# BorealisAI/noise_flow

Measured on AMD Instinct MI355X. Metric: patches/sec (32x32x4) fwd-NLL and inverse-sample; mean NLL vs CPU ref, higher is better.
Workload: dtype f32

## Files before the change

### noise_flow_amd/csrc/nf_device.h

```cpp
#pragma once
#include <stdint.h>

#define NF_MAX_OPS 64

enum : int32_t {
    NF_OP_MIX          = 1,
    NF_OP_COUPLING_FWD = 2,
    NF_OP_COUPLING_REV = 3,
    NF_OP_SDN_DIV      = 4,
    NF_OP_SDN_MUL      = 5,
    NF_OP_SCALE        = 6,
    NF_OP_SCALE_COND   = 7,
    NF_OP_STORE        = 8,
};

struct NfOp {
    int32_t type;
    int32_t off;
};

struct NfProgram {
    int32_t n_ops;
    int32_t width;
    NfOp ops[NF_MAX_OPS];
// ... 8 lines not shown
__host__ __device__ constexpr int nf_cpl_off_S(int w)  { return 64 + 36 * w + 18 * w + 2 * w + w * w; }
__host__ __device__ constexpr int nf_cpl_size(int w)   { return 64 + 36 * w + 18 * w + 2 * w + w * w + 4; }

#define NF2_MIX_SIZE 16
#define NF2_CPL_E 0
#define NF2_CPL_B1 64
#define NF2_CPL_B2 68
#define NF2_CPL_S 72
#define NF2_CPL_W1T 76
#define NF2_CPL_W2T 172
#define NF2_CPL_W3T 188
#define NF2_CPL_SIZE 332
#define NF2_MAX_FLOATS 6144

#define NF3_CPL_E 0
#define NF3_CPL_B1 64
#define NF3_CPL_B2 68
#define NF3_CPL_S 72
#define NF3_CPL_W1H 76
#define NF3_CPL_W2H 172
#define NF3_CPL_W3H 180
#define NF3_W3H_STRIDE 20
#define NF3_CPL_SIZE 260

#define NF11_CPL_E 0
#define NF11_CPL_B1 64
#define NF11_CPL_B2 68
#define NF11_CPL_S 72
#define NF11_CPL_W2H 76
#define NF11_CPL_A1 84
#define NF11_CPL_A3 340
#define NF11_CPL_SIZE 852
#define NF11_CPL_A2 852
#define NF11_CPL_SIZE_L2 1364
#define NF11_MAX_FLOATS 12288
__host__ __device__ constexpr int nf11_l1_row(int gk) { return 2 * (gk & 1) + (gk >> 1); }
__host__ __device__ constexpr int nf11_l3_row(int gk, int m3) { return 2 * (gk & 1) + m3; }
#ifndef NF11_PITCH64
#define NF11_PITCH64 80
#endif
__host__ __device__ constexpr int nf11_pitch(int side) { return side == 64 ? NF11_PITCH64 : 48; }

#define NF12_CPL_E 0
#define NF12_CPL_B1 64
#define NF12_CPL_B2 68
#define NF12_CPL_S 72
#define NF12_CPL_W2T 76
#define NF12_CPL_AOFF 92
#define NF12_CPL_SIZE 96
#define NF12_A_A1 0
#define NF12_A_A3 1536
#define NF12_A_SIZE 3072
#define NF12_PITCH 34
__host__ __device__ constexpr int nf12_col(int n) { return ((n + 12) & 15) < 8 ? 2 * ((n + 12) & 15) : 2 * (((n + 12) & 15) - 8) + 1; }
#define NF12_MAX_FLOATS 2048

#define NF4_CPL_E 0
#define NF4_CPL_S 64
#define NF4_CPL_IMG 68
#define NF4_IMG_A1 0
#define NF4_IMG_B1 768
#define NF4_IMG_A2 800
#define NF4_IMG_B2 1824
#define NF4_IMG_A3 1856
#define NF4_IMG_A3C 2880
#define NF4_IMG_SIZE 3008
#define NF4_CPL_SIZE (NF4_CPL_IMG + NF4_IMG_SIZE)
__host__ __device__ constexpr int nf4_chan(int v, int g) { return 8 * (v >> 2) + 4 * g + (v & 3); }

#define NF6_IMG_A1 0
#define NF6_IMG_B1 320
#define NF6_IMG_A2 336
#define NF6_IMG_B2 592
#define NF6_IMG_A3A 608
#define NF6_IMG_A3B 864
#define NF6_IMG_A3C 1120
#define NF6_IMG_SIZE 1184
#define NF6_CPL_SIZE (NF4_CPL_IMG + NF6_IMG_SIZE)

#define NF5_IMG_A1H 0
#define NF5_IMG_B1 512
#define NF5_IMG_A2H 544
#define NF5_IMG_B2 1056
#define NF5_IMG_A3H 1088
#define NF5_IMG_A3CH 1600
#define NF5_IMG_SIZE 1664
#define NF5_CPL_SIZE (NF4_CPL_IMG + NF5_IMG_SIZE)

#define NF7_CPL_E 0
#define NF7_CPL_S 64
#define NF7_CPL_IMG 68
__host__ __device__ constexpr int nf7_pad_width(int w) { return w <= 64 ? 64 : w <= 128 ? 128 : w <= 256 ? 256 : 512; }
__host__ __device__ constexpr int nf7_img_A1(int) { return 0; }
__host__ __device__ constexpr int nf7_img_B1(int wp) { return (wp / 32) * 768; }
__host__ __device__ constexpr int nf7_img_B2(int wp) { return (wp / 32) * 800; }
__host__ __device__ constexpr int nf7_img_A2(int wp) { return (wp / 32) * 832; }
__host__ __device__ constexpr int nf7_img_A3(int wp) { return (wp / 32) * 832 + wp * wp; }
__host__ __device__ constexpr int nf7_img_A3C(int wp) { return (wp / 32) * 832 + wp * wp + (wp / 32) * 1024; }
__host__ __device__ constexpr int nf7_img_size(int wp) { return (wp / 32) * 832 + wp * wp + (wp / 32) * (1024 + 128); }
#define NF7_P_STRIDE 44
__host__ __device__ constexpr int nf7_cpl_size(int wp) { return NF7_CPL_IMG + nf7_img_size(wp); }
#define NF7_BAND_FLOATS 32768
#define NF7_MAX_PIXELS 4096

enum : uint32_t {
    NF_K_PRIOR     = 1u,
    NF_K_PHILOX_IN = 2u,
    NF_K_FP16_CNN  = 4u,
// ... 76 lines not shown
```

### noise_flow_amd/csrc/nf_kernels.hip

```cpp
#include <hip/hip_runtime.h>
#include <math.h>
#include <stdlib.h>
#include <atomic>
#include "../../include/noiseflow_hip.h"
#include "nf_device.h"
#include "nf_dev_util.h"

#ifndef NF_PRIO
#define NF_PRIO 2
#endif
#ifndef NF_BR_SWIZZLE
#define NF_BR_SWIZZLE 1
#endif
#ifndef NF_WAVE_PRIO
#define NF_WAVE_PRIO 1
#endif
#ifndef NF_FAIR
#define NF_FAIR 1
#endif
#if NF_FAIR
#define NF_PRIO_UP()   do { } while (0)
#define NF_PRIO_DOWN() do { } while (0)
#else
#define NF_PRIO_UP()   do { if (NF_PRIO) __builtin_amdgcn_s_setprio(NF_PRIO); } while (0)
// ... 16 lines not shown
#define NF_STAMP(i) do { } while (0)
#endif

namespace {

template <int WIDTH>
__device__ __forceinline__ void stats_accumulate(const float (&h)[WIDTH], bool active, float (&s1)[WIDTH], float (&s2)[WIDTH])
{
#pragma unroll
    for (int j = 0; j < WIDTH; ++j) {
        const float v = active ? h[j] : 0.0f;
        s1[j] += v;
        s2[j] = fmaf(v, v, s2[j]);
    }
}
template <int WIDTH>
__device__ __forceinline__ void stats_direct(const float (&h)[WIDTH], bool active, double *stats, int t)
{
#pragma unroll
    for (int j = 0; j < WIDTH; ++j) {
        const float v = active ? h[j] : 0.0f;
        const float s = wave_sum(v), q = wave_sum(v * v);
        if ((t & 63) == 0) {
            atomicAdd(&stats[j], (double)s);
            atomicAdd(&stats[WIDTH + j], (double)q);
        }
    }
}
template <int WIDTH>
__device__ __forceinline__ void stats_flush(const float (&s1)[WIDTH], const float (&s2)[WIDTH], double *stats, int t)
{
#pragma unroll
    for (int j = 0; j < WIDTH; ++j) {
        const float s = wave_sum(s1[j]), q = wave_sum(s2[j]);
        if ((t & 63) == 0) {
            atomicAdd(&stats[j], (double)s);
            atomicAdd(&stats[WIDTH + j], (double)q);
        }
    }
}

__device__ __forceinline__ void nf_split3(float x0, float x1, uint32_t &h, uint32_t &m, uint32_t &l)
{
    const nf_v2bf ph = {(__bf16)x0, (__bf16)x1};
    x0 -= (float)ph[0];
    x1 -= (float)ph[1];
    const nf_v2bf pm = {(__bf16)x0, (__bf16)x1};
    x0 -= (float)pm[0];
    x1 -= (float)pm[1];
    const nf_v2bf pl = {(__bf16)x0, (__bf16)x1};
    h = __builtin_bit_cast(uint32_t, ph);
    m = __builtin_bit_cast(uint32_t, pm);
    l = __builtin_bit_cast(uint32_t, pl);
}
__device__ __forceinline__ v4f nf_mfma_bf16(const uint4 a, const uint4 b, const v4f c)
{
    return __builtin_amdgcn_mfma_f32_16x16x32_bf16(__builtin_bit_cast(nf_v8bf, a), __builtin_bit_cast(nf_v8bf, b), c, 0, 0, 0);
}

template <int WIDTH, int THREADS, int PX, bool PHILOX, bool MFMA, bool FULL, int PREC, bool BS, bool TF>
__device__ __forceinline__ void nf_flow_body(const NfProgram &prog, const NfLaunch &a)
{
    static_assert(!BS || (MFMA && PREC == 0), "the batch-statistics variant is the fp32 matrix-core kernel");
    static_assert(!TF || (FULL && MFMA && PX == 4 && PREC != 1 && !BS), "tiled full-geometry launches: the fp32 matrix-core kernel and the fp16-CNN kernel on v_mfma_f32_16x16x32_f16");
    static_assert(WIDTH % 4 == 0, "WIDTH must be a multiple of 4");
    static_assert(!MFMA || WIDTH == 4, "the matrix-core path is the width-4 specialisation");
    static_assert(PREC == 0 || (MFMA && FULL && PX == 4), "the fp16-CNN mode exists for full 2x2-blocked patches only");
    static_assert(PREC != 3 || (THREADS == 256 && !TF && !BS), "the split-bf16 mode exists for full 32x32 patches only");
    constexpr bool H16 = PREC == 1;
    constexpr bool HB = PREC == 2;
    constexpr bool SB = PREC == 3;
    constexpr bool HALF = PREC == 1 || PREC == 2;
    extern __shared__ __attribute__((aligned(16))) float smem[];

    constexpr int SIDE = THREADS * PX == 1024 ? 32 : THREADS * PX == 4096 ? 64 : 0;
    static_assert(!FULL || SIDE != 0, "FULL needs a 32x32 or 64x64 workgroup footprint");
    const int H = FULL ? SIDE : a.H, W = FULL ? SIDE : a.W, HW = H * W;
    const int Wp = SB ? NF12_PITCH : HB ? nf11_pitch(SIDE) : (H16 && SIDE == 32) ? 48 : W + 2;
    const int tile_px = ((H + 2) * Wp + 1) & ~1;
    [[maybe_unused]] const int ident_off = (a.n_params + 3) & ~3;
    constexpr bool WFIRST = HB || SB;
    constexpr int TILE_WORDS = SB ? 6 : HALF ? 3 : 2 + WIDTH;
    constexpr int RED_WORDS = (6 * (THREADS / 64) + 3) & ~3;
    float *const tiles = WFIRST ? smem + ident_off + 16 : smem;
    float2 *const t0 = reinterpret_cast<float2 *>(tiles);
    float *const th = tiles + 2 * tile_px;
    uint32_t *const t0h = reinterpret_cast<uint32_t *>(tiles);
    uint2 *const thh = reinterpret_cast<uint2 *>(tiles + tile_px);
    [[maybe_unused]] uint2 *const sr0 = reinterpret_cast<uint2 *>(tiles);
    [[maybe_unused]] uint2 *const sr1 = reinterpret_cast<uint2 *>(tiles + 2 * tile_px);
    [[maybe_unused]] uint2 *const sr2 = reinterpret_cast<uint2 *>(tiles + 4 * tile_px);
    float *const red = tiles + TILE_WORDS * tile_px;
    float *const wl = WFIRST ? smem : red + RED_WORDS;
    [[maybe_unused]] float *const bs_part = WFIRST ? red + RED_WORDS : wl + ident_off + 16;

    const int t = threadIdx.x;
    const int j4 = t & 3;
    [[maybe_unused]] bool stamp_on = true;
    [[maybe_unused]] int64_t stamp_it = 0;
    NF_STAMP(0);

    constexpr bool BLK = MFMA && FULL && PX == 4;
    const int PW = (W >> 1) + 1;
    int lidx[PX];
    int gidx[PX];
    int bmask[PX];
    bool act[PX];
    bool own[PX];
    [[maybe_unused]] int prow[PX], pcol[PX];
    int wbase = 0;
    [[maybe_unused]] int wbase3 = 0;
    if constexpr (HB || SB) {
        const int wv = t >> 6, g = (t >> 4) & 3;
        const int n = SB ? nf12_col(t & 15) : (t & 15);
        const int q = SIDE == 64 ? (wv & 1) : 0, band = SIDE == 64 ? (wv >> 1) : wv;
        const int c = 32 * q + 2 * n + (g & 1);
        wbase = (band * 8 + nf11_l1_row(g)) * Wp + 32 * q + 2 * n;
        wbase3 = (band * 8 + nf11_l3_row(g, 0)) * Wp + 32 * q + 2 * n + 2 * (g >> 1);
#pragma unroll
        for (int k = 0; k < PX; ++k) {
            const int r = band * 8 + 2 * k + (g >> 1);
            act[k] = true;
            own[k] = true;
            prow[k] = r;
            pcol[k] = c;
            gidx[k] = r * W + c;
            lidx[k] = (r + 1) * Wp + (c + 1);
            bmask[k] = (r == 0 ? 1 : 0) | (r == H - 1 ? 2 : 0) | (c == 0 ? 4 : 0) | (c == W - 1 ? 8 : 0);
        }
    } else if constexpr (BLK) {
        const int bw = W >> 1;
        int br = t / bw, bc = t - br * bw;
#if NF_BR_SWIZZLE
        if (!H16 && bw == 16) {
            br = (t >> 6) + 4 * ((t >> 4) & 3);
            bc = t & 15;
        }
#endif
        wbase = H16 ? (2 * br) * Wp + 2 * bc : (2 * br * 2) * PW + bc;
#pragma unroll
        for (int k = 0; k < PX; ++k) {
            const int dy = k >> 1, dx = k & 1;
            const int r = 2 * br + dy, c = 2 * bc + dx;
            act[k] = true;
            own[k] = true;
            prow[k] = r;
            pcol[k] = c;
            gidx[k] = r * W + c;
            lidx[k] = H16 ? (r + 1) * Wp + (c + 1) : wbase + ((dy + 1) * 2 + ((dx + 1) & 1)) * PW + ((dx + 1) >> 1);
            bmask[k] = (r == 0 ? 1 : 0) | (r == H - 1 ? 2 : 0) | (c == 0 ? 4 : 0) | (c == W - 1 ? 8 : 0);
        }
    } else {
#pragma unroll
        for (int k = 0; k < PX; ++k) {
            const int p = t + THREADS * k;
            act[k] = FULL || p < HW;
            own[k] = act[k];
            const int pp = act[k] ? p : 0;
            const int r = pp / W, c = pp - r * W;
            prow[k] = r;
            pcol[k] = c;
            gidx[k] = pp;
            lidx[k] = (r + 1) * Wp + (c + 1);
            bmask[k] = (r == 0 ? 1 : 0) | (r == H - 1 ? 2 : 0) | (c == 0 ? 4 : 0) | (c == W - 1 ? 8 : 0);
        }
    }

#ifndef NF_WSTAGE
#define NF_WSTAGE 1
#endif
    constexpr int WU = MFMA && NF_WSTAGE ? (THREADS >= 1024 ? 3 : 6) : 1;
    [[maybe_unused]] float4 wreg[WU];
    if constexpr (MFMA && NF_WSTAGE) {
        const int np4 = a.n_params >> 2;
        const float4 *const p4 = reinterpret_cast<const float4 *>(a.params);
#pragma unroll
        for (int u = 0; u < WU; ++u) {
            const int i = t + u * THREADS;
            wreg[u] = p4[i < np4 ? i : 0];
        }
    }

    float warm = 0.0f;
    float4 zin[PX];
#pragma unroll
    for (int k = 0; k < PX; ++k) zin[k] = make_float4(0.f, 0.f, 0.f, 0.f);
#ifndef NF_YPF
#define NF_YPF 1
#endif
    constexpr bool YPF = NF_YPF && MFMA && FULL && !PHILOX && THREADS == 1024 && !TF && !BS && (PREC != 0 || NF_YPF > 1);
    [[maybe_unused]] float4 yin[YPF ? PX : 1];
    [[maybe_unused]] const bool sdn_first = YPF && a.y && prog.n_ops > 0 && prog.ops[0].type == NF_OP_SDN_DIV;
    if constexpr (YPF) {
#pragma unroll
        for (int k = 0; k < PX; ++k) yin[k] = make_float4(1.f, 1.f, 1.f, 1.f);
    }
#ifndef NF_STAGGER
#define NF_STAGGER 2
#endif
#ifndef NF_STAGGER_SLEEP
#define NF_STAGGER_SLEEP 16
#endif
    const bool early = !NF_STAGGER || PHILOX || blockIdx.x < (NF_STAGGER >= 2 ? (gridDim.x >> 2) : (gridDim.x >> 1));
    bool tiled = TF;
    if constexpr (!FULL) tiled = (a.flags & NF_K_TILED) != 0;
    if ((int64_t)blockIdx.x < a.B && early && !tiled) {
        const size_t off0 = (size_t)blockIdx.x * (size_t)HW;
        if constexpr (!PHILOX) {
#pragma unroll
            for (int k = 0; k < PX; ++k)
                if (act[k]) zin[k] = reinterpret_cast<const float4 *>(a.in)[off0 + gidx[k]];
        }
        if constexpr (YPF) {
            if (sdn_first) {
#pragma unroll
                for (int k = 0; k < PX; ++k) yin[k] = reinterpret_cast<const float4 *>(a.y)[off0 + gidx[k]];
            }
        } else {
#ifndef NF_NO_WARM
#pragma unroll
        for (int k = 0; k < PX; k += NF_WARM_STEP)
            if (a.y && act[k]) warm += reinterpret_cast<const float *>(a.y)[4 * (off0 + gidx[k])];
#endif
        }
    }

    {
#ifndef NF_ZERO_BORDER
#define NF_ZERO_BORDER 0
#endif
#ifndef NF_HB_ZB
#define NF_HB_ZB 1
#endif
        if constexpr (NF_ZERO_BORDER && BLK && !HALF) {
            const int nb = 2 * (W + 2) + 2 * H;
            for (int i = t; i < nb; i += THREADS) {
                int rp, cp;
                if (i < W + 2) {
                    rp = 0;
                    cp = i;
                } else if (i < 2 * (W + 2)) {
                    rp = H + 1;
                    cp = i - (W + 2);
                } else {
                    const int j = i - 2 * (W + 2);
                    rp = 1 + (j >> 1);
                    cp = (j & 1) ? W + 1 : 0;
                }
                const int e = (rp * 2 + (cp & 1)) * PW + (cp >> 1);
                t0[e] = make_float2(0.f, 0.f);
                *reinterpret_cast<float4 *>(th + (size_t)e * 4) = make_float4(0.f, 0.f, 0.f, 0.f);
            }
        } else if constexpr (SB) {
            const int nb = 2 * (W + 2) + 2 * H;
            for (int i = t; i < nb; i += THREADS) {
                int rp, cp;
                if (i < W + 2) {
                    rp = 0;
                    cp = i;
                } else if (i < 2 * (W + 2)) {
                    rp = H + 1;
                    cp = i - (W + 2);
                } else {
                    const int j = i - 2 * (W + 2);
                    rp = 1 + (j >> 1);
                    cp = (j & 1) ? W + 1 : 0;
                }
                sr0[rp * Wp + cp] = make_uint2(0u, 0u);
                sr1[rp * Wp + cp] = make_uint2(0u, 0u);
                sr2[rp * Wp + cp] = make_uint2(0u, 0u);
            }
        } else if constexpr (NF_HB_ZB && HB) {
            const int nb = 2 * (W + 2) + 2 * H;
            for (int i = t; i < nb; i += THREADS) {
                int rp, cp;
                if (i < W + 2) {
                    rp = 0;
                    cp = i;
                } else if (i < 2 * (W + 2)) {
                    rp = H + 1;
                    cp = i - (W + 2);
                } else {
                    const int j = i - 2 * (W + 2);
                    rp = 1 + (j >> 1);
                    cp = (j & 1) ? W + 1 : 0;
                }
                t0h[rp * Wp + cp] = 0u;
                thh[rp * Wp + cp] = make_uint2(0u, 0u);
            }
        } else {
        const int nz4 = (tile_px * TILE_WORDS) >> 2;
        float4 *const s4 = reinterpret_cast<float4 *>(tiles);
        for (int i = t; i < nz4; i += THREADS) s4[i] = make_float4(0.f, 0.f, 0.f, 0.f);
        for (int i = (nz4 << 2) + t; i < tile_px * TILE_WORDS; i += THREADS) tiles[i] = 0.0f;
        }
        if (MFMA) {
            const int np4 = a.n_params >> 2;
            const float4 *const p4 = reinterpret_cast<const float4 *>(a.params);
            float4 *const w4 = reinterpret_cast<float4 *>(wl);
            if constexpr (NF_WSTAGE) {
#pragma unroll
                for (int u = 0; u < WU; ++u) {
                    const int i = t + u * THREADS;
                    if (i < np4) w4[i] = wreg[u];
                }
                for (int i = t + WU * THREADS; i < np4; i += THREADS) w4[i] = p4[i];
            } else {
                for (int i = t; i < np4; i += THREADS) w4[i] = p4[i];
            }
            for (int i = (np4 << 2) + t; i < a.n_params; i += THREADS) wl[i] = a.params[i];
            if (t < 16) wl[ident_off + t] = (t >> 2) == (t & 3) ? 1.0f : 0.0f;
        }
    }
    __syncthreads();
    asm volatile("" ::"v"(warm));
    if (NF_STAGGER && !early && (int64_t)blockIdx.x < a.B && !tiled) {
#if NF_STAGGER >= 2
        {
            const int q = (int)((blockIdx.x * 4u) / gridDim.x);
            if (q == 2) __builtin_amdgcn_s_sleep(NF_STAGGER_SLEEP);
            if (q == 3) { __builtin_amdgcn_s_sleep(NF_STAGGER_SLEEP); __builtin_amdgcn_s_sleep(NF_STAGGER_SLEEP); }
        }
#endif
        const size_t off0 = (size_t)blockIdx.x * (size_t)HW;
// ... 111 lines not shown
                const int nt = a.tile_ny * a.tile_nx;
                const int64_t img = b / nt;
                const int ti = (int)(b - img * nt);
                const int ty = ti / a.tile_nx, tx = ti - ty * a.tile_nx;
                const int oy = nf_tile_origin(ty, a.img_H, H, a.tile_halo), ox = nf_tile_origin(tx, a.img_W, W, a.tile_halo);
                const int cy0 = nf_tile_core0(ty, a.img_H, H, a.tile_halo), cy1 = nf_tile_core1(ty, a.tile_ny, a.img_H, H, a.tile_halo);
                const int cx0 = nf_tile_core0(tx, a.img_W, W, a.tile_halo), cx1 = nf_tile_core1(tx, a.tile_nx, a.img_W, W, a.tile_halo);
                patch_off = (size_t)img * (size_t)a.img_H * (size_t)a.img_W * 4u;
                patch_id = img;
#pragma unroll
                for (int k = 0; k < PX; ++k) {
                    const int r = oy + prow[k], c = ox + pcol[k];
                    gidx[k] = act[k] ? r * a.img_W + c : 0;
                    bmask[k] = (r == 0 ? 1 : 0) | (r == a.img_H - 1 ? 2 : 0) | (c == 0 ? 4 : 0) | (c == a.img_W - 1 ? 8 : 0);
                    own[k] = act[k] && r >= cy0 && r < cy1 && c >= cx0 && c < cx1;
                }
                if constexpr (!PHILOX) {
                    const float4 *in4 = reinterpret_cast<const float4 *>(a.in + patch_off);
#pragma unroll
                    for (int k = 0; k < PX; ++k) {
                        float4 v = make_float4(0.f, 0.f, 0.f, 0.f);
                        if (act[k]) v = in4[gidx[k]];
                        zin[k] = v;
                    }
                }
            }
        }

        float z[PX][4];
        if (PHILOX) {
#pragma unroll
            for (int k = 0; k < PX; ++k) {
                philox_normal4(a.seed, a.patch_base + patch_id, (uint32_t)gidx[k], NF_STREAM_SAMP, z[k]);
#pragma unroll
                for (int c = 0; c < 4; ++c) z[k][c] *= a.in_scale;
            }
        } else {
#pragma unroll
            for (int k = 0; k < PX; ++k) {
                z[k][0] = zin[k].x * a.in_scale;
                z[k][1] = zin[k].y * a.in_scale;
                z[k][2] = zin[k].z * a.in_scale;
                z[k][3] = zin[k].w * a.in_scale;
            }
        }

        float ld = 0.0f;
        if constexpr (!MFMA || BS) {
            if (a.flags & NF_K_CARRY_IN) ld = a.ld_carry[(size_t)b * THREADS + t];
        }
        float ld2 = 0.0f;
        [[maybe_unused]] int n_cpl = 0;
        [[maybe_unused]] int cpl_seen = 0;

        [[maybe_unused]] auto mix_load = [&](int moff) { return *reinterpret_cast<const float4 *>(wl + moff + 4 * j4); };
        [[maybe_unused]] auto mix_apply = [&](const float4 m) {
#pragma unroll
            for (int k = 0; k < PX; ++k) {
                v4f acc = {0.f, 0.f, 0.f, 0.f};
                acc = __builtin_amdgcn_mfma_f32_4x4x1f32(m.x, z[k][0], acc, 0, 0, 0);
                acc = __builtin_amdgcn_mfma_f32_4x4x1f32(m.y, z[k][1], acc, 0, 0, 0);
                acc = __builtin_amdgcn_mfma_f32_4x4x1f32(m.z, z[k][2], acc, 0, 0, 0);
                acc = __builtin_amdgcn_mfma_f32_4x4x1f32(m.w, z[k][3], acc, 0, 0, 0);
#pragma unroll
                for (int j = 0; j < 4; ++j) z[k][j] = acc[j];
            }
        };
        [[maybe_unused]] auto mix_mfma = [&](int mop) { mix_apply(mix_load(prog.ops[mop].off)); };

        auto sdn_apply = [&](int stype, int slot, const float4 (&yv)[PX]) {
            const float ck1 = a.cond_a[slot & 3], cb2 = a.cond_b[slot & 3];
#pragma unroll
            for (int k = 0; k < PX; ++k) {
                const float yy[4] = {yv[k].x, yv[k].y, yv[k].z, yv[k].w};
#ifndef NF_SDN_1LOG
#define NF_SDN_1LOG 1
#endif
                float rp = 1.0f;
#pragma unroll
                for (int c = 0; c < 4; ++c) {
                    const float v = fmaf(yy[c], ck1, cb2);
                    if (stype == NF_OP_SDN_DIV) {
                        const float r = __builtin_amdgcn_rsqf(v);
                        z[k][c] = z[k][c] * r;
                        if (NF_SDN_1LOG) rp = c == 0 ? r : rp * r;
                        else if (own[k]) ld = fmaf(-0.34657359027997264f, __builtin_amdgcn_logf(v), ld);
                    } else {
                        z[k][c] = z[k][c] * __builtin_amdgcn_sqrtf(v);
                    }
                }
                if (NF_SDN_1LOG && stype == NF_OP_SDN_DIV && own[k]) ld = fmaf(0.6931471805599453f, __builtin_amdgcn_logf(rp), ld);
            }
        };
        int op_begin = 0;
        if constexpr (YPF) {
            if (sdn_first) {
                float4 yv[PX];
#pragma unroll
                for (int k = 0; k < PX; ++k) yv[k] = yin[k];
                sdn_apply(NF_OP_SDN_DIV, prog.ops[0].off, yv);
                op_begin = 1;
            }
        }

        for (int op = op_begin; op < n_ops; ++op) {
            int type = prog.ops[op].type;
// ... 4 lines not shown
                    if (n_cpl == 0) { asm volatile("" ::"v"(z[0][0])); NF_STAMP(2); }
#endif
                    if (op == run_first) {
                        pr_n = run_n; pr_moff = run_moff; pr_coff = run_coff; pr_stride = run_stride;
                        type = run_type;
                    } else {
                        const int nt = op + 1 < n_ops ? prog.ops[op + 1].type : 0;
                        if (nt != NF_OP_COUPLING_FWD && nt != NF_OP_COUPLING_REV) {
                            mix_mfma(op);
                            continue;
                        }
                        pr_moff = prog.ops[op].off;
                        pr_coff = prog.ops[op + 1].off;
                        type = nt;
                    }
                    ++op;
                } else if (type == NF_OP_COUPLING_FWD || type == NF_OP_COUPLING_REV) {
                    pr_moff = ident_off;
                    pr_coff = prog.ops[op].off;
                }
            }
            [[maybe_unused]] int coff = prog.ops[op].off;
            cfloat_p P = (cfloat_p)(a.params + coff);

            if (type == NF_OP_MIX) {
                if constexpr (!MFMA) {
                    float m[16];
#pragma unroll
                    for (int i = 0; i < 16; ++i) m[i] = P[i];
#pragma unroll
                    for (int k = 0; k < PX; ++k) {
                        float o[4];
#pragma unroll
                        for (int j = 0; j < 4; ++j) {
                            float s = z[k][0] * m[j];
                            s = fmaf(z[k][1], m[4 + j], s);
                            s = fmaf(z[k][2], m[8 + j], s);
                            s = fmaf(z[k][3], m[12 + j], s);
                            o[j] = s;
                        }
#pragma unroll
                        for (int j = 0; j < 4; ++j) z[k][j] = o[j];
                    }
                }
            } else if (type == NF_OP_COUPLING_FWD || type == NF_OP_COUPLING_REV) {
                bool patch_done = false;
                synced = true;
                if constexpr (MFMA) op -= 2;
#ifndef NF_MIX_AHEAD
#define NF_MIX_AHEAD 0
#endif
                [[maybe_unused]] float4 mix_m = make_float4(0.f, 0.f, 0.f, 0.f);
                if constexpr (MFMA) mix_m = mix_load(pr_moff);
#pragma nounroll
                for (int pr_i = 0; pr_i < pr_n; ++pr_i) {
                if constexpr (MFMA) {
                    if (!NF_MIX_AHEAD) mix_m = mix_load(pr_moff);
                    mix_apply(mix_m);
                    coff = pr_coff;
                    pr_moff += pr_i + 1 < pr_n ? pr_stride : 0;
                    pr_coff += pr_stride;
                    op += 2;
                }
#if NF_FAIR
                if constexpr (MFMA && !(NF_WAVE_PRIO && THREADS == 1024)) {
                    const int lvl = (cpl_seen >= fair_t1 ? 1 : 0) + (cpl_seen >= fair_t2 ? 1 : 0) + (cpl_seen >= fair_t3 ? 1 : 0);
                    ++cpl_seen;
                    if (lvl == 0) __builtin_amdgcn_s_setprio(3);
                    else if (lvl == 1) __builtin_amdgcn_s_setprio(2);
                    else if (lvl == 2) __builtin_amdgcn_s_setprio(1);
                    else __builtin_amdgcn_s_setprio(0);
                }
#endif
#ifndef NF_HB_EARLY
#define NF_HB_EARLY 1
#endif
                [[maybe_unused]] v8h hb_a1, hb_a3a, hb_a3b, hb_a2a, hb_a2b;
                [[maybe_unused]] v4h hb_w2h;
#ifndef NF_HB_L2BIG
#define NF_HB_L2BIG 1
#endif
                constexpr bool L2B = NF_HB_L2BIG && HB && THREADS == 1024;
                [[maybe_unused]] float4 hb_b1, hb_b2, hb_e[PX];
                [[maybe_unused]] uint4 sb_a1[6], sb_a3[6];
                [[maybe_unused]] const uint4 *sb_ag = nullptr;
                if constexpr (SB) {
                    const int aoff = __builtin_amdgcn_readfirstlane(__builtin_bit_cast(int, wl[coff + NF12_CPL_AOFF]));
                    sb_ag = reinterpret_cast<const uint4 *>(a.params + aoff) + (t & 63);
#pragma unroll
                    for (int q = 0; q < 6; ++q) sb_a1[q] = sb_ag[NF12_A_A1 / 4 + 64 * q];
                    hb_b1 = *reinterpret_cast<const float4 *>(wl + coff + NF12_CPL_B1);
                    hb_b2 = *reinterpret_cast<const float4 *>(wl + coff + NF12_CPL_B2);
                }
                if constexpr (HB) {
                    const float *wb = wl + coff;
                    const uint32_t *wbw = reinterpret_cast<const uint32_t *>(wb);
                    if (NF_HB_EARLY) {
                        hb_b1 = *reinterpret_cast<const float4 *>(wb + NF11_CPL_B1);
                        hb_b2 = *reinterpret_cast<const float4 *>(wb + NF11_CPL_B2);
                        hb_a1 = __builtin_bit_cast(v8h, *reinterpret_cast<const uint4 *>(wbw + NF11_CPL_A1 + (t & 63) * 4));
                        if constexpr (L2B) {
                            hb_a2a = __builtin_bit_cast(v8h, *reinterpret_cast<const uint4 *>(wbw + NF11_CPL_A2 + (t & 63) * 4));
                            hb_a2b = __builtin_bit_cast(v8h, *reinterpret_cast<const uint4 *>(wbw + NF11_CPL_A2 + 256 + (t & 63) * 4));
                        } else {
                            hb_w2h = *reinterpret_cast<const v4h *>(wbw + NF11_CPL_W2H + j4 * 2);
                        }
                    }
                }
                if constexpr (SB) __syncthreads();
#pragma unroll
                for (int k = 0; k < PX; ++k) {
                    if constexpr (SB) {
                        uint32_t zh, zm, zl;
                        nf_split3(z[k][0], z[k][1], zh, zm, zl);
                        sr0[lidx[k]] = make_uint2(zh, zm);
                        sr1[lidx[k]] = make_uint2(zl, zh);
                    } else if constexpr (HALF) {
                        const v2h zh = {(_Float16)z[k][0], (_Float16)z[k][1]};
                        t0h[lidx[k]] = __builtin_bit_cast(uint32_t, zh);
                    } else {
                        if (act[k]) t0[lidx[k]] = make_float2(z[k][0], z[k][1]);
                    }
                }
                __syncthreads();

                if constexpr (SB) {
                    const float4 b1 = hb_b1, b2 = hb_b2;
                    const float4 w2 = *reinterpret_cast<const float4 *>(wl + coff + NF12_CPL_W2T + 4 * j4);
                    v4f h1[PX];
#pragma unroll
                    for (int k = 0; k < PX; ++k) {
                        const uint4 q00 = *reinterpret_cast<const uint4 *>(sr0 + wbase + 2 * k * Wp);
                        const uint4 q01 = *reinterpret_cast<const uint4 *>(sr0 + wbase + 2 * k * Wp + 2);
                        const uint4 q10 = *reinterpret_cast<const uint4 *>(sr1 + wbase + 2 * k * Wp);
                        const uint4 q11 = *reinterpret_cast<const uint4 *>(sr1 + wbase + 2 * k * Wp + 2);
                        v4f acc = v4f{b1.x, b1.y, b1.z, b1.w};
                        acc = nf_mfma_bf16(sb_a1[4], q10, acc);
                        acc = nf_mfma_bf16(sb_a1[5], q11, acc);
                        acc = nf_mfma_bf16(sb_a1[2], q00, acc);
                        acc = nf_mfma_bf16(sb_a1[3], q01, acc);
                        acc = nf_mfma_bf16(sb_a1[0], q00, acc);
                        acc = nf_mfma_bf16(sb_a1[1], q01, acc);
                        h1[k] = acc;
                    }
#pragma unroll
                    for (int q = 0; q < 6; ++q) sb_a3[q] = sb_ag[NF12_A_A3 / 4 + 64 * q];
                    uint2 hs[PX][3];
#pragma unroll
                    for (int k = 0; k < PX; ++k) {
                        v4f h2 = {b2.x, b2.y, b2.z, b2.w};
                        h2 = __builtin_amdgcn_mfma_f32_4x4x1f32(w2.x, nf_relu(h1[k][0]), h2, 0, 0, 0);
                        h2 = __builtin_amdgcn_mfma_f32_4x4x1f32(w2.y, nf_relu(h1[k][1]), h2, 0, 0, 0);
                        h2 = __builtin_amdgcn_mfma_f32_4x4x1f32(w2.z, nf_relu(h1[k][2]), h2, 0, 0, 0);
                        h2 = __builtin_amdgcn_mfma_f32_4x4x1f32(w2.w, nf_relu(h1[k][3]), h2, 0, 0, 0);
                        uint32_t p01[3], p23[3];
                        nf_split3(nf_relu(h2[0]), nf_relu(h2[1]), p01[0], p01[1], p01[2]);
                        nf_split3(nf_relu(h2[2]), nf_relu(h2[3]), p23[0], p23[1], p23[2]);
#pragma unroll
                        for (int q = 0; q < 3; ++q) hs[k][q] = make_uint2(p01[q], p23[q]);
                    }
#pragma unroll
                    for (int k = 0; k < PX; ++k) hb_e[k] = *reinterpret_cast<const float4 *>(wl + coff + NF12_CPL_E + 4 * bmask[k]);
                    __syncthreads();
#pragma unroll
                    for (int k = 0; k < PX; ++k) {
                        sr0[lidx[k]] = hs[k][0];
                        sr1[lidx[k]] = hs[k][1];
                        sr2[lidx[k]] = hs[k][2];
                    }
                } else if constexpr (HB) {
                    const float *wb = wl + coff;
                    const uint32_t *wbw = reinterpret_cast<const uint32_t *>(wb);
                    if (!NF_HB_EARLY) {
                        hb_b1 = *reinterpret_cast<const float4 *>(wb + NF11_CPL_B1);
                        hb_b2 = *reinterpret_cast<const float4 *>(wb + NF11_CPL_B2);
                        hb_a1 = __builtin_bit_cast(v8h, *reinterpret_cast<const uint4 *>(wbw + NF11_CPL_A1 + (t & 63) * 4));
                        if constexpr (L2B) {
                            hb_a2a = __builtin_bit_cast(v8h, *reinterpret_cast<const uint4 *>(wbw + NF11_CPL_A2 + (t & 63) * 4));
                            hb_a2b = __builtin_bit_cast(v8h, *reinterpret_cast<const uint4 *>(wbw + NF11_CPL_A2 + 256 + (t & 63) * 4));
                        } else {
                            hb_w2h = *reinterpret_cast<const v4h *>(wbw + NF11_CPL_W2H + j4 * 2);
                        }
                    }
                    const float4 b1 = hb_b1, b2 = hb_b2;
                    const v8h a1 = hb_a1;
                    [[maybe_unused]] v4h w2h = {0, 0, 0, 0};
                    if constexpr (!L2B) w2h = hb_w2h;
                    v8h bop[PX];
#pragma unroll
                    for (int k = 0; k < PX; ++k) {
                        const uint2 lo = *reinterpret_cast<const uint2 *>(t0h + wbase + 2 * k * Wp);
                        const uint2 hi = *reinterpret_cast<const uint2 *>(t0h + wbase + 2 * k * Wp + 2);
                        bop[k] = __builtin_bit_cast(v8h, make_uint4(lo.x, lo.y, hi.x, hi.y));
                    }
                    v4f h1[PX];
#pragma unroll
                    for (int k = 0; k < PX; ++k)
                        h1[k] = __builtin_amdgcn_mfma_f32_16x16x32_f16(a1, bop[k], v4f{b1.x, b1.y, b1.z, b1.w}, 0, 0, 0);
                    v4h r1[PX];
#pragma unroll
                    for (int k = 0; k < PX; ++k)
                        r1[k] = __builtin_elementwise_max(
                            v4h{(_Float16)h1[k][0], (_Float16)h1[k][1], (_Float16)h1[k][2], (_Float16)h1[k][3]}, v4h{0, 0, 0, 0});
                    v4f h2[PX];
                    if constexpr (L2B) {
#pragma unroll
                        for (int u = 0; u < PX / 2; ++u) {
                            const v8h bb = __builtin_shufflevector(r1[2 * u], r1[2 * u + 1], 0, 1, 2, 3, 4, 5, 6, 7);
                            h2[2 * u] = __builtin_amdgcn_mfma_f32_16x16x32_f16(hb_a2a, bb, v4f{b2.x, b2.y, b2.z, b2.w}, 0, 0, 0);
                            h2[2 * u + 1] = __builtin_amdgcn_mfma_f32_16x16x32_f16(hb_a2b, bb, v4f{b2.x, b2.y, b2.z, b2.w}, 0, 0, 0);
                        }
                    } else {
#pragma unroll
                    for (int k = 0; k < PX; ++k)
                        h2[k] = __builtin_amdgcn_mfma_f32_4x4x4f16(w2h, r1[k], v4f{b2.x, b2.y, b2.z, b2.w}, 0, 0, 0);
                    }
#pragma unroll
                    for (int k = 0; k < PX; ++k) {
                        const v4h r2 = __builtin_elementwise_max(
                            v4h{(_Float16)h2[k][0], (_Float16)h2[k][1], (_Float16)h2[k][2], (_Float16)h2[k][3]}, v4h{0, 0, 0, 0});
                        thh[lidx[k]] = __builtin_bit_cast(uint2, r2);
// ... 186 lines not shown
                        }
                        float h2[WIDTH];
#pragma unroll
                        for (int j = 0; j < WIDTH; ++j) h2[j] = B2[j];
#pragma unroll
                        for (int i = 0; i < WIDTH; ++i) {
                            const float hi = nf_relu(h1[k][i]);
#pragma unroll
                            for (int j = 0; j < WIDTH; ++j) h2[j] = fmaf(hi, W2[i * WIDTH + j], h2[j]);
                        }
                        if constexpr (PX > 1) {
                            if (stats_stage == 2) stats_accumulate<WIDTH>(h2, own[k], st1, st2);
                        } else {
                            if (stats_stage == 2) stats_direct<WIDTH>(h2, own[k], stats, t);
                        }
                        if (act[k]) {
                            float4 *dst = reinterpret_cast<float4 *>(th + (size_t)lidx[k] * WIDTH);
#pragma unroll
                            for (int q = 0; q < WIDTH / 4; ++q)
                                dst[q] = make_float4(nf_relu(h2[4 * q + 0]), nf_relu(h2[4 * q + 1]),
                                                     nf_relu(h2[4 * q + 2]), nf_relu(h2[4 * q + 3]));
                        }
                    }
                    if constexpr (PX > 1) {
                        if (stats_stage) stats_flush<WIDTH>(st1, st2, stats, t);
                    }
                }
                if constexpr (MFMA && NF_MIX_AHEAD) mix_m = mix_load(pr_moff);
                __syncthreads();
                if constexpr (BS) {
                    if (a.stats && op == a.stats_op && t < 8) {
                        double tot = 0.0;
#pragma unroll
                        for (int wv = 0; wv < THREADS / 64; ++wv) tot += (double)bs_part[wv * 8 + t];
                        atomicAdd(&a.stats[(blockIdx.x & (NF_STATS_SLOTS - 1)) * 8 + t], tot);
                    }
                }
                if constexpr (!MFMA || BS) {
                    if (a.stats && op == a.stats_op) {
                        patch_done = true;
                        break;
                    }
                }

                {
                    float o[PX][4];
                    float sc;
                    if constexpr (SB) {
                        sc = 0.0f;
                        uint2 *const srp[3] = {sr0, sr1, sr2};
#pragma unroll
                        for (int k = 0; k < PX; ++k) {
                            uint4 qb[3][2];
#pragma unroll
                            for (int p = 0; p < 3; ++p)
#pragma unroll
                                for (int m3 = 0; m3 < 2; ++m3) qb[p][m3] = *reinterpret_cast<const uint4 *>(srp[p] + wbase3 + (2 * k + m3) * Wp);
                            const float4 e = hb_e[k];
                            v4f acc = v4f{e.x, e.y, e.z, e.w};
                            constexpr int PA[6] = {0, 2, 1, 0, 1, 0}, PB[6] = {2, 0, 1, 1, 0, 0};
#pragma unroll
                            for (int t6 = 0; t6 < 6; ++t6)
#pragma unroll
                                for (int m3 = 0; m3 < 2; ++m3) acc = nf_mfma_bf16(sb_a3[2 * PA[t6] + m3], qb[PB[t6]][m3], acc);
#pragma unroll
                            for (int j = 0; j < 4; ++j) o[k][j] = acc[j];
                        }
                    } else if constexpr (HB) {
                        const float *wb = wl + coff;
                        const uint32_t *wbw = reinterpret_cast<const uint32_t *>(wb);
                        sc = 0.0f;
                        if (!NF_HB_EARLY) {
                            hb_a3a = __builtin_bit_cast(v8h, *reinterpret_cast<const uint4 *>(wbw + NF11_CPL_A3 + (t & 63) * 4));
                            hb_a3b = __builtin_bit_cast(v8h, *reinterpret_cast<const uint4 *>(wbw + NF11_CPL_A3 + 256 + (t & 63) * 4));
#pragma unroll
                            for (int k = 0; k < PX; ++k) hb_e[k] = *reinterpret_cast<const float4 *>(wb + NF11_CPL_E + 4 * bmask[k]);
                        }
                        const v8h a3a = hb_a3a, a3b = hb_a3b;
#ifndef NF_HB_RDAHEAD
#define NF_HB_RDAHEAD 0
#endif
                        uint4 q0[PX], q1[PX];
#pragma unroll
                        for (int k = 0; k < PX && k < NF_HB_RDAHEAD; ++k) {
                            q0[k] = *reinterpret_cast<const uint4 *>(thh + wbase3 + 2 * k * Wp);
                            q1[k] = *reinterpret_cast<const uint4 *>(thh + wbase3 + (2 * k + 1) * Wp);
                        }
                        if (NF_HB_RDAHEAD) __builtin_amdgcn_sched_barrier(0);
#pragma unroll
                        for (int k = 0; k < PX; ++k) {
                            const float4 e = hb_e[k];
                            if (k >= NF_HB_RDAHEAD) {
                                q0[k] = *reinterpret_cast<const uint4 *>(thh + wbase3 + 2 * k * Wp);
                                q1[k] = *reinterpret_cast<const uint4 *>(thh + wbase3 + (2 * k + 1) * Wp);
                            }
                            v4f acc = __builtin_amdgcn_mfma_f32_16x16x32_f16(a3a, __builtin_bit_cast(v8h, q0[k]), v4f{e.x, e.y, e.z, e.w}, 0, 0, 0);
                            acc = __builtin_amdgcn_mfma_f32_16x16x32_f16(a3b, __builtin_bit_cast(v8h, q1[k]), acc, 0, 0, 0);
#pragma unroll
                            for (int j = 0; j < 4; ++j) o[k][j] = acc[j];
                        }
                    } else if constexpr (H16) {
                        const float *wb = wl + coff;
                        const uint32_t *wbw = reinterpret_cast<const uint32_t *>(wb);
                        sc = 0.0f;
                        v4h w3h[9];
#pragma unroll
                        for (int tap = 0; tap < 8; tap += 2) {
                            const uint4 q = *reinterpret_cast<const uint4 *>(wbw + NF3_CPL_W3H + j4 * NF3_W3H_STRIDE + tap * 2);
                            w3h[tap] = __builtin_bit_cast(v4h, make_uint2(q.x, q.y));
                            w3h[tap + 1] = __builtin_bit_cast(v4h, make_uint2(q.z, q.w));
                        }
                        w3h[8] = *reinterpret_cast<const v4h *>(wbw + NF3_CPL_W3H + j4 * NF3_W3H_STRIDE + 16);
                        v4f acc[PX];
#pragma unroll
                        for (int k = 0; k < PX; ++k) {
                            const float4 e = *reinterpret_cast<const float4 *>(wb + NF3_CPL_E + 4 * bmask[k]);
                            acc[k] = v4f{e.x, e.y, e.z, e.w};
                        }
                        NF_PRIO_UP();
#pragma unroll
// ... 413 lines not shown
        const uint4 r = philox_pixel(seed, patch_base + b, p, NF_STREAM_Y);
        const float4 y = make_float4(u01_24(r.x), u01_24(r.y), u01_24(r.z), u01_24(r.w));
        if (y_out) reinterpret_cast<float4 *>(y_out)[i] = y;
        if (x_out) {
            float e[4];
            philox_normal4(seed, patch_base + b, p, NF_STREAM_XEPS, e);
            reinterpret_cast<float4 *>(x_out)[i] =
                make_float4(e[0] * sqrtf(fmaf(beta1, y.x, beta2)), e[1] * sqrtf(fmaf(beta1, y.y, beta2)),
                            e[2] * sqrtf(fmaf(beta1, y.z, beta2)), e[3] * sqrtf(fmaf(beta1, y.w, beta2)));
        }
    }
}

__global__ __launch_bounds__(64) void nf_stats_compact_kernel(const double *__restrict__ stats, int nvals, double *__restrict__ buf)
{
    const int j = threadIdx.x;
    if (j >= nvals) return;
    double s = 0.0;
    for (int k = 0; k < NF_STATS_SLOTS; ++k) s += stats[(size_t)k * nvals + j];
    buf[j] = s;
}
__global__ __launch_bounds__(64) void nf_stats_scatter_kernel(double *__restrict__ stats, int nvals, const double *__restrict__ buf)
{
    const int j = threadIdx.x;
    if (j >= nvals) return;
    stats[j] = buf[j];
    for (int k = 1; k < NF_STATS_SLOTS; ++k) stats[(size_t)k * nvals + j] = 0.0;
}

__global__ __launch_bounds__(256) void nf_eps_kernel(uint64_t seed, int64_t patch_base, int64_t B, int HW, float *__restrict__ eps_out)
{
    const int64_t total = B * (int64_t)HW;
    for (int64_t i = (int64_t)blockIdx.x * blockDim.x + threadIdx.x; i < total; i += (int64_t)gridDim.x * blockDim.x) {
        const int64_t b = i / HW;
        float e[4];
        philox_normal4(seed, patch_base + b, (uint32_t)(i - b * HW), NF_STREAM_SAMP, e);
        reinterpret_cast<float4 *>(eps_out)[i] = make_float4(e[0], e[1], e[2], e[3]);
    }
}

inline int env_int(const char *name)
{
    const char *e = getenv(name);
    return e ? atoi(e) : 0;
}

template <int WIDTH, int THREADS, int PX, bool PHILOX, bool MFMA, bool FULL, int PREC, bool BS = false, bool TF = false>
hipError_t launch_flow_p(const NfProgram &prog, const NfLaunch &a, int n_cu, hipStream_t stream)
{
    const int tile_px = ((a.H + 2) * (a.W + 2) + 1) & ~1;
    size_t lds_f = (size_t)tile_px * (PREC != 0 ? 3 : 2 + WIDTH) + ((6 * (THREADS / 64) + 3) & ~3);
    if (PREC == 1 && a.H == 32) lds_f = (size_t)(34 * 48) * 3 + ((6 * (THREADS / 64) + 3) & ~3);
    if (PREC == 2) lds_f = (size_t)((a.H + 2) * nf11_pitch(a.H)) * 3 + ((6 * (THREADS / 64) + 3) & ~3);
    if (PREC == 3) lds_f = (size_t)((a.H + 2) * NF12_PITCH) * 6 + ((6 * (THREADS / 64) + 3) & ~3);
    if (MFMA) lds_f += (size_t)((a.n_params + 3) & ~3) + 16;
    if (BS) lds_f += (size_t)(THREADS / 64) * 8 + 16;
    const size_t lds = sizeof(float) * lds_f;
    if (lds > 160 * 1024) return hipErrorInvalidValue;
    void (*const kern)(const NfProgram, const NfLaunch) = [] {
        if constexpr (TF) return &nf_flow_tile64_kernel<PHILOX, PREC>;
        else if constexpr (PREC == 3) return &nf_flow_split_kernel<PHILOX>;
        else return &nf_flow_kernel<WIDTH, THREADS, PX, PHILOX, MFMA, FULL, PREC, BS>;
    }();
    const void *fn = reinterpret_cast<const void *>(kern);
    int dev = 0;
    (void)hipGetDevice(&dev);
    static std::atomic<uint64_t> cache{0};
    const uint64_t key = ((uint64_t)(dev & 0xff) << 40) | ((uint64_t)lds << 8);
    uint64_t c = cache.load(std::memory_order_relaxed);
    int occ;
    if ((c & ~(uint64_t)0xff) == key && (c & 0xff) != 0) {
        occ = (int)(c & 0xff);
    } else {
        if (lds > 64 * 1024) {
            hipError_t e = hipFuncSetAttribute(fn, hipFuncAttributeMaxDynamicSharedMemorySize, (int)lds);
            if (e != hipSuccess) return e;
        }
        occ = 0;
        hipError_t e = hipOccupancyMaxActiveBlocksPerMultiprocessor(&occ, fn, THREADS, lds);
        if (e != hipSuccess) return e;
        if (occ < 1) occ = 1;
        if (occ > 32) occ = 32;
        cache.store(key | (uint64_t)occ, std::memory_order_relaxed);
    }
    int64_t groups = (int64_t)n_cu * occ;
    if (a.B < groups) groups = a.B;
    if (groups < 1) groups = 1;
    hipLaunchKernelGGL(kern, dim3((unsigned)groups), dim3(THREADS), lds, stream, prog, a);
    return hipGetLastError();
}

template <int WIDTH, int THREADS, int PX, bool PHILOX, bool MFMA, bool FULL>
hipError_t launch_flow_f(const NfProgram &prog, const NfLaunch &a, int n_cu, hipStream_t stream)
{
    if constexpr (MFMA && FULL && PX == 4 && THREADS == 256 && WIDTH == 4) {
        if ((a.flags & NF_K_SPLIT_BF16) && !(a.flags & (NF_K_FP16_CNN | NF_K_BATCHSTATS | NF_K_TILED)))
            return launch_flow_p<WIDTH, THREADS, PX, PHILOX, MFMA, FULL, 3>(prog, a, n_cu, stream);
    }
    if (a.flags & NF_K_SPLIT_BF16) return hipErrorInvalidValue;
    if constexpr (MFMA && FULL && PX == 4) {
        if (a.flags & NF_K_FP16_BIG) return launch_flow_p<WIDTH, THREADS, PX, PHILOX, MFMA, FULL, 2>(prog, a, n_cu, stream);
        if (a.flags & NF_K_FP16_CNN) return launch_flow_p<WIDTH, THREADS, PX, PHILOX, MFMA, FULL, 1>(prog, a, n_cu, stream);
    }
    if (a.flags & NF_K_FP16_CNN) return hipErrorInvalidValue;
    if constexpr (MFMA) {
        if (a.flags & NF_K_BATCHSTATS) return launch_flow_p<WIDTH, THREADS, PX, PHILOX, MFMA, FULL, 0, true>(prog, a, n_cu, stream);
    }
// ... 158 lines not shown
```

Measured before the change: 21.61 million.

## Remove coupling barriers in split-bf16 kernel via per-band edge row duplication

```diff
diff --git a/noise_flow_amd/csrc/nf_device.h b/noise_flow_amd/csrc/nf_device.h
--- a/noise_flow_amd/csrc/nf_device.h
+++ b/noise_flow_amd/csrc/nf_device.h
@@ -84,8 +84,10 @@
 #define NF12_A_A3 1536
 #define NF12_A_SIZE 3072
 #define NF12_PITCH 34
+#define NF12_STRIP (34 * NF12_PITCH)
+#define NF12_REGION (44 * NF12_PITCH)
 __host__ __device__ constexpr int nf12_col(int n) { return ((n + 12) & 15) < 8 ? 2 * ((n + 12) & 15) : 2 * (((n + 12) & 15) - 8) + 1; }
-#define NF12_MAX_FLOATS 2048
+#define NF12_MAX_FLOATS 1216
 
 #define NF4_CPL_E 0
 #define NF4_CPL_S 64
diff --git a/noise_flow_amd/csrc/nf_kernels.hip b/noise_flow_amd/csrc/nf_kernels.hip
--- a/noise_flow_amd/csrc/nf_kernels.hip
+++ b/noise_flow_amd/csrc/nf_kernels.hip
@@ -111,13 +111,14 @@
     constexpr bool HB = PREC == 2;
     constexpr bool SB = PREC == 3;
     constexpr bool HALF = PREC == 1 || PREC == 2;
+    constexpr bool EDGE = SB && !PHILOX;
     extern __shared__ __attribute__((aligned(16))) float smem[];
 
     constexpr int SIDE = THREADS * PX == 1024 ? 32 : THREADS * PX == 4096 ? 64 : 0;
     static_assert(!FULL || SIDE != 0, "FULL needs a 32x32 or 64x64 workgroup footprint");
     const int H = FULL ? SIDE : a.H, W = FULL ? SIDE : a.W, HW = H * W;
     const int Wp = SB ? NF12_PITCH : HB ? nf11_pitch(SIDE) : (H16 && SIDE == 32) ? 48 : W + 2;
-    const int tile_px = ((H + 2) * Wp + 1) & ~1;
+    const int tile_px = SB ? NF12_REGION : ((H + 2) * Wp + 1) & ~1;
     [[maybe_unused]] const int ident_off = (a.n_params + 3) & ~3;
     constexpr bool WFIRST = HB || SB;
     constexpr int TILE_WORDS = SB ? 6 : HALF ? 3 : 2 + WIDTH;
@@ -150,6 +151,7 @@
     [[maybe_unused]] int prow[PX], pcol[PX];
     int wbase = 0;
     [[maybe_unused]] int wbase3 = 0;
+    [[maybe_unused]] int sb_d = 0;
     if constexpr (HB || SB) {
         const int wv = t >> 6, g = (t >> 4) & 3;
         const int n = SB ? nf12_col(t & 15) : (t & 15);
@@ -157,6 +159,7 @@
         const int c = 32 * q + 2 * n + (g & 1);
         wbase = (band * 8 + nf11_l1_row(g)) * Wp + 32 * q + 2 * n;
         wbase3 = (band * 8 + nf11_l3_row(g, 0)) * Wp + 32 * q + 2 * n + 2 * (g >> 1);
+        if constexpr (EDGE) sb_d = NF12_STRIP - 6 * Wp * __builtin_amdgcn_readfirstlane(band);
 #pragma unroll
         for (int k = 0; k < PX; ++k) {
             const int r = band * 8 + 2 * k + (g >> 1);
@@ -244,6 +247,16 @@
     const bool early = !NF_STAGGER || PHILOX || blockIdx.x < (NF_STAGGER >= 2 ? (gridDim.x >> 2) : (gridDim.x >> 1));
     bool tiled = TF;
     if constexpr (!FULL) tiled = (a.flags & NF_K_TILED) != 0;
+#ifndef NF12_AWARM
+#define NF12_AWARM 0
+#endif
+    if constexpr (SB && NF12_AWARM) {
+        int ncpl = 0;
+        for (int i = 0; i < prog.n_ops; ++i) ncpl += (prog.ops[i].type == NF_OP_COUPLING_FWD || prog.ops[i].type == NF_OP_COUPLING_REV);
+        const int nlines = ncpl * (NF12_A_SIZE * 4 / 128), step = gridDim.x >= 8 ? (int)(gridDim.x >> 3) : 1;
+        const float *const aimg = a.params + a.n_params;
+        for (int i = (int)(blockIdx.x >> 3) + step * t; i < nlines; i += step * THREADS) warm += aimg[32 * i];
+    }
     if ((int64_t)blockIdx.x < a.B && early && !tiled) {
         const size_t off0 = (size_t)blockIdx.x * (size_t)HW;
         if constexpr (!PHILOX) {
@@ -310,6 +323,11 @@
                 sr1[rp * Wp + cp] = make_uint2(0u, 0u);
                 sr2[rp * Wp + cp] = make_uint2(0u, 0u);
             }
+            constexpr int SQ = 10 * NF12_PITCH / 2;
+            for (int i = t; EDGE && i < 3 * SQ; i += THREADS) {
+                const int p = i / SQ;
+                *reinterpret_cast<uint4 *>(sr0 + p * tile_px + NF12_STRIP + 2 * (i - p * SQ)) = make_uint4(0u, 0u, 0u, 0u);
+            }
         } else if constexpr (NF_HB_ZB && HB) {
             const int nb = 2 * (W + 2) + 2 * H;
             for (int i = t; i < nb; i += THREADS) {
@@ -692,7 +710,7 @@
                         }
                     }
                 }
-                if constexpr (SB) __syncthreads();
+                if constexpr (SB && !EDGE) __syncthreads();
 #pragma unroll
                 for (int k = 0; k < PX; ++k) {
                     if constexpr (SB) {
@@ -746,12 +764,13 @@
                     }
 #pragma unroll
                     for (int k = 0; k < PX; ++k) hb_e[k] = *reinterpret_cast<const float4 *>(wl + coff + NF12_CPL_E + 4 * bmask[k]);
-                    __syncthreads();
+                    if constexpr (!EDGE) __syncthreads();
 #pragma unroll
                     for (int k = 0; k < PX; ++k) {
-                        sr0[lidx[k]] = hs[k][0];
-                        sr1[lidx[k]] = hs[k][1];
-                        sr2[lidx[k]] = hs[k][2];
+                        const int e = lidx[k] + (!EDGE ? 0 : k == 0 ? ((t & 32) ? 0 : sb_d) : k == PX - 1 ? ((t & 32) ? sb_d - 6 * Wp : 0) : 0);
+                        sr0[e] = hs[k][0];
+                        sr1[e] = hs[k][1];
+                        sr2[e] = hs[k][2];
                     }
                 } else if constexpr (HB) {
                     const float *wb = wl + coff;
@@ -1044,10 +1063,12 @@
 #pragma unroll
                         for (int k = 0; k < PX; ++k) {
                             uint4 qb[3][2];
+                            const int rb = wbase3 + 2 * k * Wp +
+                                           (!EDGE ? 0 : k == 0 ? ((t & 16) ? 0 : sb_d) : k == PX - 1 ? ((t & 16) ? sb_d - 6 * Wp : 0) : 0);
 #pragma unroll
                             for (int p = 0; p < 3; ++p)
 #pragma unroll
-                                for (int m3 = 0; m3 < 2; ++m3) qb[p][m3] = *reinterpret_cast<const uint4 *>(srp[p] + wbase3 + (2 * k + m3) * Wp);
+                                for (int m3 = 0; m3 < 2; ++m3) qb[p][m3] = *reinterpret_cast<const uint4 *>(srp[p] + rb + m3 * Wp);
                             const float4 e = hb_e[k];
                             v4f acc = v4f{e.x, e.y, e.z, e.w};
                             constexpr int PA[6] = {0, 2, 1, 0, 1, 0}, PB[6] = {2, 0, 1, 1, 0, 0};
@@ -1577,7 +1598,9 @@
     size_t lds_f = (size_t)tile_px * (PREC != 0 ? 3 : 2 + WIDTH) + ((6 * (THREADS / 64) + 3) & ~3);
     if (PREC == 1 && a.H == 32) lds_f = (size_t)(34 * 48) * 3 + ((6 * (THREADS / 64) + 3) & ~3);
     if (PREC == 2) lds_f = (size_t)((a.H + 2) * nf11_pitch(a.H)) * 3 + ((6 * (THREADS / 64) + 3) & ~3);
-    if (PREC == 3) lds_f = (size_t)((a.H + 2) * NF12_PITCH) * 6 + ((6 * (THREADS / 64) + 3) & ~3);
+    if (PREC == 3) lds_f = (size_t)NF12_REGION * 6 + ((6 * (THREADS / 64) + 3) & ~3);
+    static_assert(sizeof(float) * (NF12_REGION * 6 + ((6 * 4 + 3) & ~3) + NF12_MAX_FLOATS + 16) <= 40 * 1024,
+                  "split-bf16: 4 workgroups per CU at the largest LDS part the host accepts");
     if (MFMA) lds_f += (size_t)((a.n_params + 3) & ~3) + 16;
     if (BS) lds_f += (size_t)(THREADS / 64) * 8 + 16;
     const size_t lds = sizeof(float) * lds_f;
```

Measured after the change: 21.75 million, median of 6. No clear change (+0.6%).

## Prefetch split-bf16 coupling weights via buffer loads and hoist z splitting

Applied to the files above, without the earlier changes.

```diff
diff --git a/noise_flow_amd/csrc/nf_kernels.hip b/noise_flow_amd/csrc/nf_kernels.hip
--- a/noise_flow_amd/csrc/nf_kernels.hip
+++ b/noise_flow_amd/csrc/nf_kernels.hip
@@ -92,6 +92,28 @@
     h = __builtin_bit_cast(uint32_t, ph);
     m = __builtin_bit_cast(uint32_t, pm);
     l = __builtin_bit_cast(uint32_t, pl);
+}
+#ifndef NF_SB_SPLIT
+#define NF_SB_SPLIT 1
+#endif
+__device__ __forceinline__ void nf_split3_min(float x0, float x1, uint32_t &h, uint32_t &m, uint32_t &l)
+{
+    h = __builtin_bit_cast(uint32_t, nf_v2bf{(__bf16)x0, (__bf16)x1});
+    asm("" : "+v"(h));
+    x0 -= __builtin_bit_cast(float, h << 16);
+    x1 -= __builtin_bit_cast(float, h & 0xffff0000u);
+    asm("" : "+v"(x0), "+v"(x1));
+    m = __builtin_bit_cast(uint32_t, nf_v2bf{(__bf16)x0, (__bf16)x1});
+    asm("" : "+v"(m));
+    x0 -= __builtin_bit_cast(float, m << 16);
+    x1 -= __builtin_bit_cast(float, m & 0xffff0000u);
+    asm("" : "+v"(x0), "+v"(x1));
+    l = __builtin_bit_cast(uint32_t, nf_v2bf{(__bf16)x0, (__bf16)x1});
+}
+__device__ __forceinline__ void nf_split3_sb(float x0, float x1, uint32_t &h, uint32_t &m, uint32_t &l)
+{
+    if (NF_SB_SPLIT) nf_split3_min(x0, x1, h, m, l);
+    else nf_split3(x0, x1, h, m, l);
 }
 __device__ __forceinline__ v4f nf_mfma_bf16(const uint4 a, const uint4 b, const v4f c)
 {
@@ -527,6 +549,7 @@
         float ld2 = 0.0f;
         [[maybe_unused]] int n_cpl = 0;
         [[maybe_unused]] int cpl_seen = 0;
+        [[maybe_unused]] int cpl_ord = 0;
 
         [[maybe_unused]] auto mix_load = [&](int moff) { return *reinterpret_cast<const float4 *>(wl + moff + 4 * j4); };
         [[maybe_unused]] auto mix_apply = [&](const float4 m) {
@@ -637,6 +660,23 @@
 #endif
                 [[maybe_unused]] float4 mix_m = make_float4(0.f, 0.f, 0.f, 0.f);
                 if constexpr (MFMA) mix_m = mix_load(pr_moff);
+#ifndef NF_SB_APF
+#define NF_SB_APF 1
+#endif
+                [[maybe_unused]] uint4 sb_a1[6];
+                [[maybe_unused]] int sb_aoff = 0;
+                [[maybe_unused]] auto sb_load = [&](uint4 (&dst)[6], int off) {
+                    const __amdgpu_buffer_rsrc_t rs = __builtin_amdgcn_make_buffer_rsrc(const_cast<float *>(a.params), 0, 0x7fffffff, 0x00020000);
+                    const int lane_b = (t & 63) * 16;
+#pragma unroll
+                    for (int q = 0; q < 6; ++q)
+                        dst[q] = __builtin_bit_cast(uint4, __builtin_amdgcn_raw_buffer_load_b128(rs, lane_b, off * 4 + 1024 * q, 0));
+                };
+                if constexpr (SB) {
+                    sb_aoff = a.n_params + cpl_ord * NF12_A_SIZE;
+                    cpl_ord += pr_n;
+                    if (NF_SB_APF) sb_load(sb_a1, sb_aoff + NF12_A_A1);
+                }
 #pragma nounroll
                 for (int pr_i = 0; pr_i < pr_n; ++pr_i) {
                 if constexpr (MFMA) {
@@ -667,13 +707,9 @@
 #endif
                 constexpr bool L2B = NF_HB_L2BIG && HB && THREADS == 1024;
                 [[maybe_unused]] float4 hb_b1, hb_b2, hb_e[PX];
-                [[maybe_unused]] uint4 sb_a1[6], sb_a3[6];
-                [[maybe_unused]] const uint4 *sb_ag = nullptr;
+                [[maybe_unused]] uint4 sb_a3[6];
                 if constexpr (SB) {
-                    const int aoff = __builtin_amdgcn_readfirstlane(__builtin_bit_cast(int, wl[coff + NF12_CPL_AOFF]));
-                    sb_ag = reinterpret_cast<const uint4 *>(a.params + aoff) + (t & 63);
-#pragma unroll
-                    for (int q = 0; q < 6; ++q) sb_a1[q] = sb_ag[NF12_A_A1 / 4 + 64 * q];
+                    if (!NF_SB_APF) sb_load(sb_a1, sb_aoff + NF12_A_A1);
                     hb_b1 = *reinterpret_cast<const float4 *>(wl + coff + NF12_CPL_B1);
                     hb_b2 = *reinterpret_cast<const float4 *>(wl + coff + NF12_CPL_B2);
                 }
@@ -692,14 +728,23 @@
                         }
                     }
                 }
-                if constexpr (SB) __syncthreads();
+#ifndef NF_SB_ZEARLY
+#define NF_SB_ZEARLY 1
+#endif
+                [[maybe_unused]] uint32_t zs[PX][3];
+                if constexpr (SB) {
+                    if (NF_SB_ZEARLY) {
+#pragma unroll
+                        for (int k = 0; k < PX; ++k) nf_split3_sb(z[k][0], z[k][1], zs[k][0], zs[k][1], zs[k][2]);
+                    }
+                    __syncthreads();
+                }
 #pragma unroll
                 for (int k = 0; k < PX; ++k) {
                     if constexpr (SB) {
-                        uint32_t zh, zm, zl;
-                        nf_split3(z[k][0], z[k][1], zh, zm, zl);
-                        sr0[lidx[k]] = make_uint2(zh, zm);
-                        sr1[lidx[k]] = make_uint2(zl, zh);
+                        if (!NF_SB_ZEARLY) nf_split3_sb(z[k][0], z[k][1], zs[k][0], zs[k][1], zs[k][2]);
+                        sr0[lidx[k]] = make_uint2(zs[k][0], zs[k][1]);
+                        sr1[lidx[k]] = make_uint2(zs[k][2], zs[k][0]);
                     } else if constexpr (HALF) {
                         const v2h zh = {(_Float16)z[k][0], (_Float16)z[k][1]};
                         t0h[lidx[k]] = __builtin_bit_cast(uint32_t, zh);
@@ -728,8 +773,7 @@
                         acc = nf_mfma_bf16(sb_a1[1], q01, acc);
                         h1[k] = acc;
                     }
-#pragma unroll
-                    for (int q = 0; q < 6; ++q) sb_a3[q] = sb_ag[NF12_A_A3 / 4 + 64 * q];
+                    sb_load(sb_a3, sb_aoff + NF12_A_A3);
                     uint2 hs[PX][3];
 #pragma unroll
                     for (int k = 0; k < PX; ++k) {
@@ -739,8 +783,8 @@
                         h2 = __builtin_amdgcn_mfma_f32_4x4x1f32(w2.z, nf_relu(h1[k][2]), h2, 0, 0, 0);
                         h2 = __builtin_amdgcn_mfma_f32_4x4x1f32(w2.w, nf_relu(h1[k][3]), h2, 0, 0, 0);
                         uint32_t p01[3], p23[3];
-                        nf_split3(nf_relu(h2[0]), nf_relu(h2[1]), p01[0], p01[1], p01[2]);
-                        nf_split3(nf_relu(h2[2]), nf_relu(h2[3]), p23[0], p23[1], p23[2]);
+                        nf_split3_sb(nf_relu(h2[0]), nf_relu(h2[1]), p01[0], p01[1], p01[2]);
+                        nf_split3_sb(nf_relu(h2[2]), nf_relu(h2[3]), p23[0], p23[1], p23[2]);
 #pragma unroll
                         for (int q = 0; q < 3; ++q) hs[k][q] = make_uint2(p01[q], p23[q]);
                     }
@@ -1058,6 +1102,8 @@
 #pragma unroll
                             for (int j = 0; j < 4; ++j) o[k][j] = acc[j];
                         }
+                        if (pr_i + 1 < pr_n) sb_aoff += NF12_A_SIZE;
+                        if (NF_SB_APF) sb_load(sb_a1, sb_aoff + NF12_A_A1);
                     } else if constexpr (HB) {
                         const float *wb = wl + coff;
                         const uint32_t *wbw = reinterpret_cast<const uint32_t *>(wb);
```

After: 21.38 million before, 22.09 million after (median of 6 runs). 1.03x the previous value.
